# zenghjian/SceneSplat

Measured on AMD Instinct MI355X. Metric: Gaussians/s encoder fwd+bwd, 102k-pt chunks, higher is better.
Workload: dtype bf16

## Files before the change

### include/scenesplat_hip.h

```cpp
#ifndef SCENESPLAT_HIP_H
#define SCENESPLAT_HIP_H
#include <stddef.h>
#include <stdint.h>

#ifdef __cplusplus
extern "C" {
#endif

struct ihipStream_t;
typedef struct ihipStream_t* ss_stream_t;

#define SS_MAX_ORDERS 8
enum { SS_ORDER_Z = 0, SS_ORDER_Z_TRANS = 1, SS_ORDER_HILBERT = 2, SS_ORDER_HILBERT_TRANS = 3 };
enum { SS_DTYPE_F32 = 0, SS_DTYPE_BF16 = 1 };
enum { SS_ATTN_SIMT = 0, SS_ATTN_MFMA = 1 };

int ss_version(void);

int ss_serialize_encode(const int32_t* grid_coord, const int32_t* batch, int64_t n, int depth, const int* orders,
                        int num_orders, int64_t* codes, ss_stream_t stream);
int ss_offsets_to_batch(const int32_t* offsets, int num_batches, int64_t n, int32_t* batch, ss_stream_t stream);
int ss_count_duplicates(const int64_t* sorted_keys, int64_t n, int32_t* count, ss_stream_t stream);
int ss_grid_coord_max(const int32_t* grid_coord, int64_t n, int32_t* out_max, ss_stream_t stream);
size_t ss_argsort_workspace_bytes(int64_t n, int num_segments);
// ... 10 lines not shown
                        int32_t* grid_coord_out, int32_t* batch_out, int64_t* codes_out, ss_stream_t stream);
int ss_batch_offsets(const int32_t* batch, const int32_t* perm, int64_t n, int num_batches, int32_t* offsets,
                     ss_stream_t stream);

int ss_window_index(const int32_t* order, const int32_t* offsets, const int32_t* offsets_pad, int num_batches,
                    int patch_size, int64_t n_pad, int32_t* gidx, int32_t* sidx, ss_stream_t stream);
int ss_window_attn_fwd(const void* qkv, const int32_t* gidx, const int32_t* sidx, const int32_t* win_start,
                       int num_windows, int max_window, int64_t n, int64_t n_pad, int channels, int num_heads,
                       float scale, int dtype, int impl, void* out, float* lse, ss_stream_t stream);
size_t ss_window_attn_bwd_workspace_bytes(int64_t n, int64_t n_pad, int channels, int num_heads, int dtype);
int ss_window_attn_bwd(const void* qkv, const void* out, const void* dout, const float* lse, const int32_t* gidx,
                       const int32_t* sidx, const int32_t* win_start, int num_windows, int max_window, int64_t n,
                       int64_t n_pad, int channels, int num_heads, float scale, int dtype, int impl, void* dqkv,
                       void* workspace, size_t workspace_bytes, ss_stream_t stream);

int ss_cast_bf16_group(const int64_t* desc, const int32_t* wg_start, int nprob, int total_workgroups, ss_stream_t stream);
int ss_cast_bf16_group_elems_per_workgroup(void);

int ss_row_keep_scales(const int64_t* seed, const float* keep, float* out, int64_t n, ss_stream_t stream);

int ss_gelu(const void* x, const void* dy, void* out, int64_t numel, int dtype, ss_stream_t stream);

int ss_stream_capture_status(ss_stream_t stream);
unsigned long long ss_stream_capture_id(ss_stream_t stream);

int ss_linear_fwd_headmajor(const void* x, const int32_t* row_index, const void* weight, const float* bias, void* out_hm,
                            int64_t m, int k, int n_out, int channels, int head_dim, float sec0_scale, ss_stream_t stream);
int ss_headmajor_pack(const void* src, int in_dtype, const int32_t* gidx, void* hm, int64_t n_pad, int channels,
                      int num_heads, int sections, float sec0_scale, ss_stream_t stream);
int ss_window_attn_hm_fwd(const void* hm, const int32_t* sidx, const int32_t* win_start, int num_windows, int max_window,
                          int64_t n, int64_t n_pad, int channels, int num_heads, void* out, float* neg_lse2,
                          ss_stream_t stream);
size_t ss_window_attn_hm_bwd_workspace_bytes(int64_t n, int64_t n_pad, int channels, int num_heads);
int ss_window_attn_hm_bwd(const void* hm, const void* out, const void* dout, const float* neg_lse2, const int32_t* gidx,
                          const int32_t* sidx, const int32_t* win_start, int num_windows, int max_window, int64_t n,
                          int64_t n_pad, int channels, int num_heads, float scale, void* dqkv, void* workspace,
                          size_t workspace_bytes, ss_stream_t stream);

int ss_subm_rulebook(const int32_t* grid_coord, const int32_t* batch, int64_t n, int depth,
                     const int64_t* zkeys_sorted, const int32_t* zorder, int swap_xy, int kernel_size, int32_t* nbr,
                     ss_stream_t stream);
int ss_subm_tap_mask_keys(const int32_t* nbr, const int32_t* order, int64_t n, int taps, int coarse_bits, int64_t* keys,
                          ss_stream_t stream);
int64_t ss_subm_rulebook_table_size(int64_t n);
int ss_subm_rulebook_hashed(const int32_t* grid_coord, const int32_t* batch, int64_t n, int depth, int kernel_size, int32_t* nbr,
                            void* workspace, size_t workspace_bytes, ss_stream_t stream);

int ss_subm_conv_fwd(const void* in, const void* weight, const float* bias, const int32_t* nbr, const int32_t* rowperm,
                     void* out, int64_t n, int cin, int cout, int taps, int out_dtype, ss_stream_t stream);
int ss_subm_weight_mirror(const void* w, void* wt, int cout, int taps, int cin, ss_stream_t stream);
int ss_stream_create_cu_mask(int nwords, const uint32_t* mask, void** stream_out);
int ss_subm_im2col(const void* src, const int32_t* nbr, void* dst, int64_t n, int taps, int64_t row_bytes, ss_stream_t stream);
int ss_gemm8_ok(int64_t m, int k, int n, int taps);
int ss_subm_conv_fwd_pipe(const void* in, const void* weight, const float* bias, const int32_t* nbr, const int32_t* rowperm,
                          void* out, int64_t n, int cin, int cout, int taps, int out_dtype, ss_stream_t stream);
int ss_subm_conv_fwd_pipe_walk(const void* in, const void* weight, const float* bias, const int32_t* nbr_walk, const int32_t* rowperm,
                               void* out, int64_t n, int cin, int cout, int taps, int out_dtype, ss_stream_t stream);
int ss_subm_conv_fwd_uses_pipe(int64_t n, int cin, int cout, int taps);
int ss_subm_conv_fwd_walk(const void* in, const void* weight, const float* bias, const int32_t* nbr, const int32_t* nbr_walk,
                          const int32_t* rowperm, void* out, int64_t n, int cin, int cout, int taps, int out_dtype, ss_stream_t stream);
int ss_linear_fwd(const void* x, const void* weight, const float* bias, void* out, int64_t m, int k, int n, int out_dtype,
                  ss_stream_t stream);
int ss_wgrad_xcd_order(void);
int ss_wgrad_set_xcd_order(int on);
int ss_wgrad8_ok(int64_t n, int cin, int cout, int taps);
int ss_subm_conv_wgrad_pipe(const void* in, const void* dout, const int32_t* nbr, const int32_t* rowperm,
                            const int32_t* blk_count, const int32_t* blk_list, float* dweight, int64_t n, int cin, int cout,
                            int taps, ss_stream_t stream);
int ss_linear_wgrad(const void* x, const void* dy, float* dweight, float* dbias, int64_t m, int k_in, int n_out,
                    ss_stream_t stream);
int ss_linear_wgrad_group_plan(int64_t m, int k_in, int n_out, int64_t* desc_words);
int ss_linear_wgrad_tiles(int k_in, int n_out);
int ss_linear_wgrad_group_plan2(int64_t m, int k_in, int n_out, int launch_tiles, int64_t* desc_words);
int ss_linear_wgrad_group(const int64_t* desc, const int32_t* wg_start, int nprob, int total_workgroups, ss_stream_t stream);
int ss_subm_conv_splits(int64_t n, int cout, int taps);
int ss_subm_conv_fwd_splitk(const void* in, const void* weight, const float* bias, const int32_t* nbr, const int32_t* rowperm,
                            float* acc32, int64_t n, int cin, int cout, int taps, int splits, ss_stream_t stream);
int ss_subm_block_lists(const int32_t* nbr, const int32_t* rowperm, int64_t n, int taps, int32_t* blk_count,
                        int32_t* blk_list, ss_stream_t stream);
int ss_subm_conv_wgrad(const void* in, const void* dout, const int32_t* nbr, const int32_t* rowperm,
                       const int32_t* blk_count, const int32_t* blk_list, float* dweight, int64_t n, int cin, int cout,
                       int taps, ss_stream_t stream);

int ss_subm_f32_ok(int cin_padded, int cout);
int ss_subm_f32_fwd(const float* in, const float* wq, const float* bias, const int32_t* nbr_walk, const int32_t* rowperm,
                    float* out, int64_t n, int cin_padded, int cout, int taps, ss_stream_t stream);
int ss_subm_f32_dgrad_dup(const float* dout_folded, const float* wq, const int32_t* nbr_walk, const int32_t* rowperm, float* din,
                          int64_t n, int cin_padded, int cout, int taps, ss_stream_t stream);
int ss_subm_f32_wgrad(const float* in, const float* dout, const int32_t* nbr_walk, const int32_t* rowperm,
                      const int32_t* blk_count, const int32_t* blk_list, float* dweight, int64_t n, int cin_padded,
                      int cin, int cout, int taps, ss_stream_t stream);

int ss_subm_conv_wgrad_pipe_walk(const void* in, const void* dout, const int32_t* nbr_walk, const int32_t* rowperm,
                                 const int32_t* blk_count, const int32_t* blk_list, float* dweight, int64_t n, int cin, int cout,
                                 int taps, ss_stream_t stream);
int ss_subm_conv_wgrad_uses_pipe(int64_t n, int cin, int cout, int taps);
int ss_subm_conv_wgrad_walk(const void* in, const void* dout, const int32_t* nbr, const int32_t* nbr_walk, const int32_t* rowperm,
                            const int32_t* blk_count, const int32_t* blk_list, float* dweight, int64_t n, int cin, int cout,
                            int taps, ss_stream_t stream);

int ss_add_layernorm_fwd(const void* x, int x_dtype, const void* y, int y_dtype, const float* rowscale,
                         const float* gamma, const float* beta, float eps, void* xout, int xout_dtype, void* xcopy_bf16,
                         void* h, int h_dtype, float* mean, float* rstd, int64_t n, int channels, ss_stream_t stream);
int ss_ln_add_ln_fwd(const void* x, int x_dtype, const void* t, int t_dtype, const float* gamma0, const float* beta0, float eps0,
                     const float* gamma1, const float* beta1, float eps1, float* xout, void* h, int h_dtype, float* stats,
                     int64_t n, int channels, ss_stream_t stream);
// ... 117 lines not shown
```

### scenesplat_amd/_lib.py

```python
import ctypes
import os

import torch

_HERE = os.path.dirname(os.path.abspath(__file__))
LIB_PATH = os.path.join(_HERE, "lib", "libscenesplat_hip.so")

c_p = ctypes.c_void_p
c_i = ctypes.c_int
c_i64 = ctypes.c_int64
c_f = ctypes.c_float
c_sz = ctypes.c_size_t

PROTOTYPES = {
    "ss_version": (c_i, []),
    "ss_serialize_encode": (c_i, [c_p, c_p, c_i64, c_i, ctypes.POINTER(c_i), c_i, c_p, c_p]),
    "ss_offsets_to_batch": (c_i, [c_p, c_i, c_i64, c_p, c_p]),
    "ss_count_duplicates": (c_i, [c_p, c_i64, c_p, c_p]),
    "ss_grid_coord_max": (c_i, [c_p, c_i64, c_p, c_p]),
    "ss_argsort_workspace_bytes": (c_sz, [c_i64, c_i]),
    "ss_argsort_i64": (c_i, [c_p, c_i, c_i64, c_i, c_p, c_p, c_p, c_p, c_sz, c_p]),
    "ss_pool_partition_workspace_bytes": (c_sz, [c_i64]),
    "ss_pool_partition": (c_i, [c_p, c_p, c_i64, c_i, c_p, c_p, c_p, c_p, c_p, c_sz, c_p]),
    "ss_pool_level_attrs": (c_i, [c_p, c_i64, c_i64, c_p, c_p, c_p, c_i, c_i, c_p, c_p, c_p, c_p]),
    "ss_batch_offsets": (c_i, [c_p, c_p, c_i64, c_i, c_p, c_p]),
    "ss_window_index": (c_i, [c_p, c_p, c_p, c_i, c_i, c_i64, c_p, c_p, c_p]),
    "ss_window_attn_fwd": (c_i, [c_p, c_p, c_p, c_p, c_i, c_i, c_i64, c_i64, c_i, c_i, c_f, c_i, c_i, c_p, c_p, c_p]),
    "ss_window_attn_bwd_workspace_bytes": (c_sz, [c_i64, c_i64, c_i, c_i, c_i]),
    "ss_window_attn_bwd": (c_i, [c_p, c_p, c_p, c_p, c_p, c_p, c_p, c_i, c_i, c_i64, c_i64, c_i, c_i, c_f, c_i, c_i,
                                 c_p, c_p, c_sz, c_p]),
    "ss_gelu": (c_i, [c_p, c_p, c_p, c_i64, c_i, c_p]),
    "ss_row_keep_scales": (c_i, [c_p, c_p, c_p, c_i64, c_p]),
    "ss_stream_capture_status": (c_i, [c_p]),
    "ss_stream_capture_id": (ctypes.c_ulonglong, [c_p]),
    "ss_cast_bf16_group": (c_i, [c_p, c_p, c_i, c_i, c_p]),
    "ss_cast_bf16_group_elems_per_workgroup": (c_i, []),
    "ss_linear_fwd_headmajor": (c_i, [c_p, c_p, c_p, c_p, c_p, c_i64, c_i, c_i, c_i, c_i, c_f, c_p]),
    "ss_headmajor_pack": (c_i, [c_p, c_i, c_p, c_p, c_i64, c_i, c_i, c_i, c_f, c_p]),
    "ss_window_attn_hm_fwd": (c_i, [c_p, c_p, c_p, c_i, c_i, c_i64, c_i64, c_i, c_i, c_p, c_p, c_p]),
    "ss_window_attn_hm_bwd_workspace_bytes": (c_sz, [c_i64, c_i64, c_i, c_i]),
    "ss_window_attn_hm_bwd": (c_i, [c_p, c_p, c_p, c_p, c_p, c_p, c_p, c_i, c_i, c_i64, c_i64, c_i, c_i, c_f, c_p, c_p, c_sz, c_p]),
    "ss_subm_rulebook": (c_i, [c_p, c_p, c_i64, c_i, c_p, c_p, c_i, c_i, c_p, c_p]),
    "ss_subm_conv_fwd": (c_i, [c_p, c_p, c_p, c_p, c_p, c_p, c_i64, c_i, c_i, c_i, c_i, c_p]),
    "ss_stream_create_cu_mask": (c_i, [c_i, c_p, c_p]),
    "ss_ln_add_ln_fwd": (c_i, [c_p, c_i, c_p, c_i, c_p, c_p, c_f, c_p, c_p, c_f, c_p, c_p, c_i, c_p, c_i64, c_i, c_p]),
    "ss_ln_add_ln_bwd": (c_i, [c_p, c_p, c_i, c_p, c_p, c_i, c_p, c_p, c_p, c_p, c_i, c_p, c_i, c_p, c_i64, c_i, c_i, c_p]),
    "ss_segment_minmax": (c_i, [c_p, c_p, c_p, c_p, c_p, c_i64, c_i, c_i, c_i, c_p]),
    "ss_segment_minmax_bwd": (c_i, [c_p, c_p, c_p, c_i64, c_i, c_i, c_p]),
    "ss_subm_rulebook_table_size": (c_i64, [c_i64]),
    "ss_subm_rulebook_hashed": (c_i, [c_p, c_p, c_i64, c_i, c_i, c_p, c_p, ctypes.c_size_t, c_p]),
    "ss_subm_tap_mask_keys": (c_i, [c_p, c_p, c_i64, c_i, c_i, c_p, c_p]),
    "ss_subm_weight_mirror": (c_i, [c_p, c_p, c_i, c_i, c_i, c_p]),
    "ss_subm_im2col": (c_i, [c_p, c_p, c_p, c_i64, c_i, c_i64, c_p]),
    "ss_gemm8_ok": (c_i, [c_i64, c_i, c_i, c_i]),
    "ss_subm_conv_fwd_pipe": (c_i, [c_p, c_p, c_p, c_p, c_p, c_p, c_i64, c_i, c_i, c_i, c_i, c_p]),
    "ss_linear_fwd": (c_i, [c_p, c_p, c_p, c_p, c_i64, c_i, c_i, c_i, c_p]),
    "ss_wgrad_xcd_order": (c_i, []),
    "ss_wgrad_set_xcd_order": (c_i, [c_i]),
    "ss_wgrad8_ok": (c_i, [c_i64, c_i, c_i, c_i]),
    "ss_subm_conv_wgrad_pipe": (c_i, [c_p, c_p, c_p, c_p, c_p, c_p, c_p, c_i64, c_i, c_i, c_i, c_p]),
    "ss_linear_wgrad": (c_i, [c_p, c_p, c_p, c_p, c_i64, c_i, c_i, c_p]),
    "ss_linear_wgrad_group_plan": (c_i, [c_i64, c_i, c_i, c_p]),
    "ss_linear_wgrad_tiles": (c_i, [c_i, c_i]),
    "ss_linear_wgrad_group_plan2": (c_i, [c_i64, c_i, c_i, c_i, c_p]),
    "ss_linear_wgrad_group": (c_i, [c_p, c_p, c_i, c_i, c_p]),
    "ss_subm_conv_splits": (c_i, [c_i64, c_i, c_i]),
    "ss_subm_conv_fwd_splitk": (c_i, [c_p, c_p, c_p, c_p, c_p, c_p, c_i64, c_i, c_i, c_i, c_i, c_p]),
    "ss_subm_block_lists": (c_i, [c_p, c_p, c_i64, c_i, c_p, c_p, c_p]),
    "ss_subm_conv_wgrad": (c_i, [c_p, c_p, c_p, c_p, c_p, c_p, c_p, c_i64, c_i, c_i, c_i, c_p]),
    "ss_subm_conv_fwd_pipe_walk": (c_i, [c_p, c_p, c_p, c_p, c_p, c_p, c_i64, c_i, c_i, c_i, c_i, c_p]),
    "ss_subm_conv_fwd_uses_pipe": (c_i, [c_i64, c_i, c_i, c_i]),
    "ss_subm_conv_fwd_walk": (c_i, [c_p, c_p, c_p, c_p, c_p, c_p, c_p, c_i64, c_i, c_i, c_i, c_i, c_p]),
    "ss_subm_conv_wgrad_pipe_walk": (c_i, [c_p, c_p, c_p, c_p, c_p, c_p, c_p, c_i64, c_i, c_i, c_i, c_p]),
    "ss_subm_conv_wgrad_uses_pipe": (c_i, [c_i64, c_i, c_i, c_i]),
    "ss_subm_conv_wgrad_walk": (c_i, [c_p, c_p, c_p, c_p, c_p, c_p, c_p, c_p, c_i64, c_i, c_i, c_i, c_p]),
    "ss_subm_f32_ok": (c_i, [c_i, c_i]),
    "ss_subm_f32_fwd": (c_i, [c_p, c_p, c_p, c_p, c_p, c_p, c_i64, c_i, c_i, c_i, c_p]),
    "ss_subm_f32_dgrad_dup": (c_i, [c_p, c_p, c_p, c_p, c_p, c_i64, c_i, c_i, c_i, c_p]),
    "ss_dup_fold_rows": (c_i, [c_p, c_p, c_p, c_p, c_i64, c_i, c_i, c_p]),
    "ss_dup_zero_rows": (c_i, [c_p, c_p, c_p, c_i64, c_i64, c_p]),
    "ss_subm_f32_wgrad": (c_i, [c_p, c_p, c_p, c_p, c_p, c_p, c_p, c_i64, c_i, c_i, c_i, c_i, c_p]),
    "ss_add_layernorm_fwd": (c_i, [c_p, c_i, c_p, c_i, c_p, c_p, c_p, c_f, c_p, c_i, c_p, c_p, c_i, c_p, c_p, c_i64, c_i, c_p]),
    "ss_add_layernorm_bwd_blocks": (c_i, [c_i64]),
    "ss_group_partial_sums_outputs_per_workgroup": (c_i, []),
    "ss_group_partial_sums": (c_i, [c_p, c_p, c_i, c_i, c_p]),
    "ss_transpose16_group": (c_i, [c_p, c_p, c_i, c_i, c_p]),
    "ss_subm_weight_mirror_group_tile": (c_i, []),
    "ss_subm_weight_mirror_group": (c_i, [c_p, c_p, c_i, c_i, c_p]),
    "ss_add_layernorm_bwd": (c_i, [c_p, c_i, c_p, c_i, c_p, c_i, c_p, c_i, c_p, c_p, c_p, c_p, c_p, c_i, c_p, c_i, c_p, c_p,
                                   c_i64, c_i, c_i, c_p]),
    "ss_col_stats": (c_i, [c_p, c_i, c_p, c_p, c_p, c_i64, c_i, c_i, c_p]),
    "ss_bn_stats_finish": (c_i, [c_p, c_p, c_i, c_i, c_i64, c_f, c_f, c_p, c_p, c_p, c_p, c_p, c_p]),
    "ss_bn_bwd_finish": (c_i, [c_p, c_i, c_i, c_i64, c_p, c_p, c_p]),
    "ss_bn_act_fwd": (c_i, [c_p, c_i, c_p, c_p, c_p, c_p, c_i, c_p, c_i, c_i64, c_i, c_p]),
    "ss_bn_act_bwd_reduce": (c_i, [c_p, c_i, c_p, c_i, c_p, c_p, c_p, c_p, c_i, c_p, c_p, c_i64, c_i, c_i, c_p]),
    "ss_bn_act_bwd_apply": (c_i, [c_p, c_i, c_p, c_i, c_p, c_p, c_p, c_p, c_i, c_p, c_p, c_p, c_i, c_i64, c_i, c_p]),
    "ss_feat_text_scan": (c_i, [c_p, c_p, c_i64, c_i, c_i, c_p, c_p, c_p, c_p, c_p]),
    "ss_lang_head_blocks": (c_i, [c_i64]),
    "ss_lang_head_fwd": (c_i, [c_p, c_i, c_p, c_i, c_p, c_i, c_p, c_i, c_p, c_p, c_p, c_i64, c_i, c_p]),
    "ss_lang_head_bwd": (c_i, [c_p, c_i, c_p, c_i, c_p, c_i, c_p, c_p, c_p, c_i, c_p, c_i, c_i64, c_i, c_p]),
    "ss_seg_loss_workspace_bytes": (c_sz, [c_i64, c_i]),
    "ss_seg_loss_fwd": (c_i, [c_p, c_i, c_p, c_i64, c_i, c_i64, c_p, c_i, c_p, c_p, c_p, c_p, c_p, c_sz, c_p]),
    "ss_seg_loss_bwd": (c_i, [c_p, c_i, c_p, c_i64, c_i, c_i64, c_p, c_p, c_p, c_p, c_p, c_p]),
    "ss_seg_iou": (c_i, [c_p, c_i, c_p, c_p, c_i64, c_i, c_i64, c_p, c_p]),
    "ss_gather_rows": (c_i, [c_p, c_p, c_p, c_i64, c_i64, c_p]),
    "ss_scatter_rows": (c_i, [c_p, c_p, c_p, c_i64, c_i64, c_p]),
    "ss_gather_add_rows": (c_i, [c_p, c_p, c_p, c_p, c_i64, c_i, c_i, c_p]),
# ... 65 lines not shown
```

### scenesplat_amd/build.py

```python
import glob
import os
import subprocess
import sys

HERE = os.path.dirname(os.path.abspath(__file__))
CSRC = os.path.join(HERE, "csrc")
LIBDIR = os.path.join(HERE, "lib")
LIB = os.path.join(LIBDIR, "libscenesplat_hip.so")
HEADER = os.path.join(os.path.dirname(HERE), "include", "scenesplat_hip.h")


def sources():
    return sorted(glob.glob(os.path.join(CSRC, "*.hip")))


def _headers():
    return glob.glob(os.path.join(CSRC, "*.h")) + [HEADER]


def needs_build():
    if not os.path.exists(LIB):
        return True
    t = os.path.getmtime(LIB)
    return any(os.path.getmtime(d) > t for d in sources() + _headers())


def build(force=False, verbose=True):
    os.makedirs(LIBDIR, exist_ok=True)
    if os.environ.get("SS_EXTRA_HIPCC_FLAGS"):
        force = True
    if not force and not needs_build():
        return LIB
    hipcc = os.environ.get("HIPCC", "/opt/rocm/bin/hipcc")
    objdir = os.path.join(LIBDIR, "obj")
    os.makedirs(objdir, exist_ok=True)
    hdr_t = max(os.path.getmtime(h) for h in _headers())
    objs, procs = [], []
    for src in sources():
        obj = os.path.join(objdir, os.path.basename(src)[:-4] + ".o")
        objs.append(obj)
        if not force and os.path.exists(obj) and os.path.getmtime(obj) > max(os.path.getmtime(src), hdr_t):
            continue
        cmd = [hipcc, "--offload-arch=gfx950", "-O3", "-std=c++17", "-fPIC", "-c", src, "-o", obj,
               "-Wno-unused-value", "-Wno-unused-result",
               "-mllvm", "-amdgpu-mfma-vgpr-form"] + os.environ.get("SS_EXTRA_HIPCC_FLAGS", "").split()
        if verbose:
            print(" ".join(cmd), flush=True)
        procs.append((src, subprocess.Popen(cmd)))
    for src, p in procs:
        if p.wait() != 0:
            raise RuntimeError(f"hipcc failed on {src}")
    cmd = [hipcc, "--offload-arch=gfx950", "-shared", "-fPIC", "-o", LIB] + objs
    if verbose:
        print(" ".join(cmd), flush=True)
    subprocess.check_call(cmd)
    return LIB


if __name__ == "__main__":
    build(force="--force" in sys.argv)
```

### scenesplat_amd/csrc/gemm8.hip

```cpp
#include "common.h"
#include <stdlib.h>
#include "../../include/scenesplat_hip.h"

typedef __attribute__((ext_vector_type(8))) __bf16 g8_bf8_t;
#define G8_MFMA(a, b, c) __builtin_amdgcn_mfma_f32_16x16x32_bf16((a), (b), (c), 0, 0, 0)
#define G8_TAPS_MAX 27
#define G8_ZERO_ELEMS 4096

#ifndef G8_STAGGER
#define G8_STAGGER 1
#endif
#define G8_BUF 65536
#define G8_HALF 16384
#define G8_OFF_B 32768
#define G8_OFF_NBR 131072
#define G8_OFF_ROWID (G8_OFF_NBR + G8_TAPS_MAX * 256 * 4)
#define G8_OFF_MASK (G8_OFF_ROWID + 1024)
#define G8_LDS_BYTES (G8_OFF_MASK + 16)

__device__ uint4 g8_zero[G8_ZERO_ELEMS / 8];

__device__ __forceinline__ void g8_glds16(const void* gsrc, char* lds_wave_base) {
  __builtin_amdgcn_global_load_lds((const __attribute__((address_space(1))) void*)gsrc,
                                   (__attribute__((address_space(3))) void*)lds_wave_base, 16, 0, 0);
}
__device__ __forceinline__ g8_bf8_t g8_lds(const char* p) {
  return __builtin_bit_cast(g8_bf8_t, *reinterpret_cast<const uint4*>(p));
}

template <bool GATHER, typename OutT, bool HM = false>
__global__ void __launch_bounds__(512)
k_gemm8(const unsigned short* __restrict__ A, const unsigned short* __restrict__ W, const float* __restrict__ bias,
        const int32_t* __restrict__ nbr, const int32_t* __restrict__ rowperm, OutT* __restrict__ out, int M, int K,
        int N, int taps, int ntn, int hm_c = 0, int hm_d = 0, float hm_scale = 1.f, int walk = 0) {
  __shared__ __attribute__((aligned(16))) char smem[G8_LDS_BYTES];
  int32_t* nbr_s = reinterpret_cast<int32_t*>(smem + G8_OFF_NBR);
  int32_t* rowid_s = reinterpret_cast<int32_t*>(smem + G8_OFF_ROWID);
  unsigned* mask_s = reinterpret_cast<unsigned*>(smem + G8_OFF_MASK);
  const int tid = threadIdx.x, wave = tid >> 6, lane = tid & 63, lq = lane & 15, g = lane >> 4;
  const int wr = wave >> 2, wc = wave & 3;
  int L;
  {
    const int nwg = gridDim.x, orig = blockIdx.x, xcd = orig & 7, q = nwg >> 3, r = nwg & 7;
    L = (xcd < r ? xcd * (q + 1) : r * (q + 1) + (xcd - r) * q) + (orig >> 3);
  }
  const int m0 = (L / ntn) * 256, n0 = (L % ntn) * 256;

  unsigned rem = 0u;
  int tap = 0;
  if (GATHER) {
    if (tid < 256) {
      int k = m0 + tid;
      rowid_s[tid] = k < M ? (rowperm ? rowperm[k] : k) : -1;
    }
    if (tid == 0) *mask_s = 0u;
// ... 174 lines not shown
    asm volatile("s_waitcnt vmcnt(0)" ::: "memory");
  }

  int64_t hm_base[2][2];
  float hm_mul[2][2];
  if (HM) {
#pragma unroll
    for (int hb = 0; hb < 2; ++hb)
#pragma unroll
      for (int ni = 0; ni < 2; ++ni) {
        const int col = min(n0 + 64 * wc + 32 * hb + 16 * ni + 4 * g, N - 4);
        const int sec = col / hm_c, cc = col - sec * hm_c, hd = cc / hm_d, dd = cc - hd * hm_d;
        hm_base[hb][ni] = ((int64_t)sec * (hm_c / hm_d) + hd) * M * hm_d + dd;
        hm_mul[hb][ni] = sec == 0 ? hm_scale : 1.f;
      }
  }
#pragma unroll
  for (int ha = 0; ha < 2; ++ha)
#pragma unroll
    for (int mi = 0; mi < 4; ++mi) {
      const int R = 128 * wr + 64 * ha + 16 * mi + lq;
      int64_t row;
      if (GATHER) { row = rowid_s[R]; } else { row = m0 + R < M ? m0 + R : -1; }
      if (row < 0) continue;
#pragma unroll
      for (int hb = 0; hb < 2; ++hb)
#pragma unroll
        for (int ni = 0; ni < 2; ++ni) {
          const int col = n0 + 64 * wc + 32 * hb + 16 * ni + 4 * g;
          if (col >= N) continue;
          f32x4_t v = acc[ha][mi][hb][ni];
          if (bias) { float4 bv = *reinterpret_cast<const float4*>(bias + col); v[0] += bv.x; v[1] += bv.y; v[2] += bv.z; v[3] += bv.w; }
          OutT* op = out + row * N + col;
          if (HM) {
            const float m_ = hm_mul[hb][ni];
            v[0] *= m_; v[1] *= m_; v[2] *= m_; v[3] *= m_;
            op = out + hm_base[hb][ni] + row * hm_d;
          }
          if (sizeof(OutT) == 2) {
            uint2 u; u.x = pack_bf16x2(v[0], v[1]); u.y = pack_bf16x2(v[2], v[3]);
            *reinterpret_cast<uint2*>(op) = u;
          } else {
            *reinterpret_cast<float4*>(op) = make_float4(v[0], v[1], v[2], v[3]);
          }
        }
    }
}

extern "C" int ss_gemm8_ok(int64_t m, int k, int n, int taps) {
  return m > 0 && m < (1LL << 31) && k >= 64 && (k & 63) == 0 && k <= G8_ZERO_ELEMS && n >= 4 && (n & 3) == 0 &&
         taps >= 1 && taps <= G8_TAPS_MAX;
}

template <bool GATHER>
static int g8_launch(const void* a, const void* w, const float* bias, const int32_t* nbr, const int32_t* rowperm, void* out,
                     int64_t m, int k, int n, int taps, int out_dtype, hipStream_t stream, int walk = 0) {
  if (!ss_gemm8_ok(m, k, n, taps)) return SS_ERR_ARG;
  const int ntm = ss_div_up(m, 256), ntn = ss_div_up(n, 256);
  dim3 grid(ntm * ntn), block(512);
  const unsigned short* A = (const unsigned short*)a; const unsigned short* Wp = (const unsigned short*)w;
  if (out_dtype == SS_BF16)
    SS_LAUNCH((k_gemm8<GATHER, unsigned short>), grid, block, 0, stream, A, Wp, bias, nbr, rowperm, (unsigned short*)out, (int)m, k, n, taps, ntn, 0, 0, 1.f, walk);
  else if (out_dtype == SS_F32)
    SS_LAUNCH((k_gemm8<GATHER, float>), grid, block, 0, stream, A, Wp, bias, nbr, rowperm, (float*)out, (int)m, k, n, taps, ntn, 0, 0, 1.f, walk);
  else
    return SS_ERR_ARG;
  return SS_OK;
}

extern "C" int ss_subm_conv_fwd_pipe(const void* in, const void* weight, const float* bias, const int32_t* nbr,
                                     const int32_t* rowperm, void* out, int64_t n, int cin, int cout, int taps,
                                     int out_dtype, hipStream_t stream) {
  if (n == 0) return SS_OK;
  return g8_launch<true>(in, weight, bias, nbr, rowperm, out, n, cin, cout, taps, out_dtype, stream);
}

extern "C" int ss_subm_conv_fwd_pipe_walk(const void* in, const void* weight, const float* bias, const int32_t* nbr_walk,
                                          const int32_t* rowperm, void* out, int64_t n, int cin, int cout, int taps,
                                          int out_dtype, hipStream_t stream) {
  if (n == 0) return SS_OK;
  return g8_launch<true>(in, weight, bias, nbr_walk, rowperm, out, n, cin, cout, taps, out_dtype, stream, 1);
}

extern "C" int ss_linear_fwd(const void* x, const void* weight, const float* bias, void* out, int64_t m, int k, int n,
                             int out_dtype, hipStream_t stream) {
  if (m == 0) return SS_OK;
  return g8_launch<false>(x, weight, bias, nullptr, nullptr, out, m, k, n, 1, out_dtype, stream);
}

extern "C" int ss_linear_fwd_headmajor(const void* x, const int32_t* row_index, const void* weight, const float* bias,
                                       void* out_hm, int64_t m, int k, int n_out, int channels, int head_dim,
                                       float sec0_scale, hipStream_t stream) {
  if (m == 0) return SS_OK;
  if (!ss_gemm8_ok(m, k, n_out, 1) || channels <= 0 || head_dim <= 0 || (head_dim & 3) || channels % head_dim || n_out % channels ||
      !row_index)
    return SS_ERR_ARG;
  const int ntm = ss_div_up(m, 256), ntn = ss_div_up(n_out, 256);
  dim3 grid(ntm * ntn), block(512);
  SS_LAUNCH((k_gemm8<false, unsigned short, true>), grid, block, 0, stream, (const unsigned short*)x, (const unsigned short*)weight,
            bias, (const int32_t*)nullptr, row_index, (unsigned short*)out_hm, (int)m, k, n_out, 1, ntn, channels, head_dim,
            sec0_scale);
  return SS_OK;
}
```

### scenesplat_amd/native.py

```python
import ctypes
import os

import torch

from . import _lib
from ._lib import check

F32, BF16 = 0, 1
ATTN_SIMT, ATTN_MFMA = 0, 1
HAVE_MFMA_ATTN = True
ORDER_IDS = {"z": 0, "z-trans": 1, "hilbert": 2, "hilbert-trans": 3}


_GROUP_WIDE_SHARES = os.environ.get("SS_WGRAD_GROUP_WIDE", "1") != "0"
_GROUP_KEEP = []
_GROUP_LOCK = __import__("threading").Lock()


class DescriptorPool:

    def __init__(self, nbytes=1 << 20):
        self.buf = torch.empty(int(nbytes), dtype=torch.uint8).pin_memory()
        self.off = 0
        self.device_side = []
# ... 195 lines not shown
    return keys


def subm_conv_fwd_uses_pipe(n, cin, cout, taps):
    return bool(lib().ss_subm_conv_fwd_uses_pipe(n, cin, cout, taps)) and lib().ss_subm_conv_splits(n, cout, taps) <= 1


def subm_conv_fwd(x, w, bias, nbr, rowperm, out_dtype=torch.bfloat16, nbr_walk=None):
    n, cin = x.shape
    cout, taps, cin2 = w.shape
    _req(x, torch.bfloat16, "x"); _req(w, torch.bfloat16, "w"); _req(nbr, torch.int32, "nbr", (taps, n))
    if cin2 != cin or cin % 8:
        raise RuntimeError(f"subm_conv_fwd: cin mismatch / not a multiple of 8 ({cin}, {cin2})")
    if bias is not None:
        _req(bias, torch.float32, "bias", (cout,))
    if rowperm is not None:
        _req(rowperm, torch.int32, "rowperm", (n,))
    splits = lib().ss_subm_conv_splits(n, cout, taps)
    if splits > 1:
        acc = torch.zeros((n, cout), dtype=torch.float32, device=x.device)
        check(lib().ss_subm_conv_fwd_splitk(_p(x), _p(w), _p(bias), _p(nbr), _p(rowperm), _p(acc), n, cin, cout, taps, splits,
                                            _stream()), "ss_subm_conv_fwd_splitk")
        return acc if out_dtype == torch.float32 else acc.to(out_dtype)
    out = torch.empty((n, cout), dtype=out_dtype, device=x.device)
    if nbr_walk is not None:
        _req(nbr_walk, torch.int32, "nbr_walk", (taps, n))
        check(lib().ss_subm_conv_fwd_walk(_p(x), _p(w), _p(bias), _p(nbr), _p(nbr_walk), _p(rowperm), _p(out), n, cin, cout, taps,
                                          dtype_code(out), _stream()), "ss_subm_conv_fwd_walk")
        return out
    check(lib().ss_subm_conv_fwd(_p(x), _p(w), _p(bias), _p(nbr), _p(rowperm), _p(out), n, cin, cout, taps,
                                 dtype_code(out), _stream()), "ss_subm_conv_fwd")
    return out


def subm_weight_mirror(w):
    cout, taps, cin = w.shape
    _req(w, torch.bfloat16, "w")
    wt = torch.empty((cin, taps, cout), dtype=torch.bfloat16, device=w.device)
    check(lib().ss_subm_weight_mirror(_p(w), _p(wt), cout, taps, cin, _stream()), "ss_subm_weight_mirror")
    return wt


def subm_im2col(x, nbr):
    n, c = x.shape
    taps = nbr.shape[0]
    _req(x, torch.bfloat16, "x"); _req(nbr, torch.int32, "nbr", (taps, n))
    if c % 8:
        raise RuntimeError("subm_im2col: channels must be a multiple of 8")
    out = torch.empty((n, taps * c), dtype=torch.bfloat16, device=x.device)
    check(lib().ss_subm_im2col(_p(x), _p(nbr), _p(out), n, taps, c * 2, _stream()), "ss_subm_im2col")
    return out


def subm_conv_fwd_pipe(x, w, bias, nbr, rowperm, out_dtype=torch.bfloat16):
    n, cin = x.shape
    cout, taps = w.shape[0], w.shape[1]
    out = torch.empty((n, cout), dtype=out_dtype, device=x.device)
    check(lib().ss_subm_conv_fwd_pipe(_p(x), _p(w), _p(bias), _p(nbr), _p(rowperm), _p(out), n, cin, cout, taps,
                                      dtype_code(out), _stream()), "ss_subm_conv_fwd_pipe")
    return out


def linear_fwd(x, w, bias=None, out_dtype=torch.bfloat16):
    m, k = x.shape
    n = w.shape[0]
    out = torch.empty((m, n), dtype=out_dtype, device=x.device)
    check(lib().ss_linear_fwd(_p(x), _p(w), _p(bias), _p(out), m, k, n, dtype_code(out), _stream()), "ss_linear_fwd")
    return out


def subm_block_lists(nbr, rowperm):
    taps, n = nbr.shape
    _req(nbr, torch.int32, "nbr")
    if rowperm is not None:
        _req(rowperm, torch.int32, "rowperm", (n,))
    nb = (n + 63) // 64
    cnt = torch.empty(taps, dtype=torch.int32, device=nbr.device)
    lst = torch.empty((taps, nb), dtype=torch.int32, device=nbr.device)
    check(lib().ss_subm_block_lists(_p(nbr), _p(rowperm), n, taps, _p(cnt), _p(lst), _stream()), "ss_subm_block_lists")
    return cnt, lst


_ARENA = {"buf": None, "off": 0}


def zero_arena_begin(numel, device):
    _ARENA["buf"] = torch.zeros(int(numel), dtype=torch.float32, device=device) if numel > 0 else None
    _ARENA["off"] = 0


def zeros_f32(numel, device):
    buf, off = _ARENA["buf"], _ARENA["off"]
    if buf is not None and buf.device == device and off + numel <= buf.numel():
        _ARENA["off"] = off + ((numel + 3) & ~3)
        return buf[off:off + numel]
    return torch.zeros(int(numel), dtype=torch.float32, device=device)


def subm_conv_wgrad(x, dout, nbr, rowperm, blocks, out=None, nbr_walk=None):
    n, cin = x.shape
    cout = dout.shape[1]
    taps = nbr.shape[0]
    _req(x, torch.bfloat16, "x"); _req(dout, torch.bfloat16, "dout", (n, cout)); _req(nbr, torch.int32, "nbr", (taps, n))
    if cin % 8 or cout % 8:
        raise RuntimeError("subm_conv_wgrad: channels must be multiples of 8")
    if rowperm is not None:
        _req(rowperm, torch.int32, "rowperm", (n,))
    dw = zeros_f32(cout * taps * cin, x.device).view(cout, taps, cin) if out is None else _req(out, torch.float32, "out", (cout, taps, cin))
    cnt, lst = blocks
    _req(cnt, torch.int32, "blk_count", (taps,)); _req(lst, torch.int32, "blk_list", (taps, (n + 63) // 64))
    if nbr_walk is not None:
        _req(nbr_walk, torch.int32, "nbr_walk", (taps, n))
    check(lib().ss_subm_conv_wgrad_walk(_p(x), _p(dout), _p(nbr), _p(nbr_walk), _p(rowperm), _p(cnt), _p(lst), _p(dw), n, cin, cout, taps,
# ... 655 lines not shown
```

Before: 2.827 million.

## Add 4-wave 256x256 gemm8 variant with AGPR accumulators for large convs

Adds a new 256-thread (4-wave) GEMM kernel in which each wave holds a 128x128 accumulator tile in AGPRs. It uses a hand-scheduled double-buffered LDS pipeline with global_load_lds DMA interleaved between MFMAs, and the file is compiled without the VGPR-form MFMA flag. By default, gathered sparse-conv forward calls with m>=25600 and k>=512 go to the new kernel; other calls can be forced to 4 or 8 waves through an env var or setter. The aim is to cut LDS and synchronisation overhead per MFMA and to improve latency hiding in the big conv GEMMs. The cost is heavy register pressure and a fragile, hand-tuned schedule.

```diff
diff --git a/include/scenesplat_hip.h b/include/scenesplat_hip.h
--- a/include/scenesplat_hip.h
+++ b/include/scenesplat_hip.h
@@ -86,6 +86,8 @@
 int ss_stream_create_cu_mask(int nwords, const uint32_t* mask, void** stream_out);
 int ss_subm_im2col(const void* src, const int32_t* nbr, void* dst, int64_t n, int taps, int64_t row_bytes, ss_stream_t stream);
 int ss_gemm8_ok(int64_t m, int k, int n, int taps);
+int ss_gemm8_waves(void);
+int ss_gemm8_set_waves(int waves);
 int ss_subm_conv_fwd_pipe(const void* in, const void* weight, const float* bias, const int32_t* nbr, const int32_t* rowperm,
                           void* out, int64_t n, int cin, int cout, int taps, int out_dtype, ss_stream_t stream);
 int ss_subm_conv_fwd_pipe_walk(const void* in, const void* weight, const float* bias, const int32_t* nbr_walk, const int32_t* rowperm,
diff --git a/scenesplat_amd/_lib.py b/scenesplat_amd/_lib.py
--- a/scenesplat_amd/_lib.py
+++ b/scenesplat_amd/_lib.py
@@ -53,6 +53,8 @@
     "ss_subm_weight_mirror": (c_i, [c_p, c_p, c_i, c_i, c_i, c_p]),
     "ss_subm_im2col": (c_i, [c_p, c_p, c_p, c_i64, c_i, c_i64, c_p]),
     "ss_gemm8_ok": (c_i, [c_i64, c_i, c_i, c_i]),
+    "ss_gemm8_waves": (c_i, []),
+    "ss_gemm8_set_waves": (c_i, [c_i]),
     "ss_subm_conv_fwd_pipe": (c_i, [c_p, c_p, c_p, c_p, c_p, c_p, c_i64, c_i, c_i, c_i, c_i, c_p]),
     "ss_linear_fwd": (c_i, [c_p, c_p, c_p, c_p, c_i64, c_i, c_i, c_i, c_p]),
     "ss_wgrad_xcd_order": (c_i, []),
diff --git a/scenesplat_amd/build.py b/scenesplat_amd/build.py
--- a/scenesplat_amd/build.py
+++ b/scenesplat_amd/build.py
@@ -8,6 +8,9 @@
 LIBDIR = os.path.join(HERE, "lib")
 LIB = os.path.join(LIBDIR, "libscenesplat_hip.so")
 HEADER = os.path.join(os.path.dirname(HERE), "include", "scenesplat_hip.h")
+
+
+AGPR_FORM = {"gemm8w4.hip"}
 
 
 def sources():
@@ -42,8 +45,10 @@
         if not force and os.path.exists(obj) and os.path.getmtime(obj) > max(os.path.getmtime(src), hdr_t):
             continue
         cmd = [hipcc, "--offload-arch=gfx950", "-O3", "-std=c++17", "-fPIC", "-c", src, "-o", obj,
-               "-Wno-unused-value", "-Wno-unused-result",
-               "-mllvm", "-amdgpu-mfma-vgpr-form"] + os.environ.get("SS_EXTRA_HIPCC_FLAGS", "").split()
+               "-Wno-unused-value", "-Wno-unused-result"]
+        if os.path.basename(src) not in AGPR_FORM:
+            cmd += ["-mllvm", "-amdgpu-mfma-vgpr-form"]
+        cmd += os.environ.get("SS_EXTRA_HIPCC_FLAGS", "").split()
         if verbose:
             print(" ".join(cmd), flush=True)
         procs.append((src, subprocess.Popen(cmd)))
diff --git a/scenesplat_amd/csrc/gemm8.hip b/scenesplat_amd/csrc/gemm8.hip
--- a/scenesplat_amd/csrc/gemm8.hip
+++ b/scenesplat_amd/csrc/gemm8.hip
@@ -1,6 +1,7 @@
 #include "common.h"
 #include <stdlib.h>
 #include "../../include/scenesplat_hip.h"
+#include "gemm8w4.h"
 
 typedef __attribute__((ext_vector_type(8))) __bf16 g8_bf8_t;
 #define G8_MFMA(a, b, c) __builtin_amdgcn_mfma_f32_16x16x32_bf16((a), (b), (c), 0, 0, 0)
@@ -281,10 +282,30 @@
          taps >= 1 && taps <= G8_TAPS_MAX;
 }
 
+enum { G8_CLS_CONV = 0, G8_CLS_PLAIN = 1, G8_CLS_HM = 2 };
+static int g8_waves_mode = -1;
+extern "C" int ss_gemm8_waves(void) {
+  if (g8_waves_mode < 0) { const char* e = getenv("SS_GEMM8_WAVES"); const int v = e ? atoi(e) : 0; g8_waves_mode = (v == 4 || v == 8) ? v : 0; }
+  return g8_waves_mode;
+}
+extern "C" int ss_gemm8_set_waves(int waves) {
+  if (waves != 0 && waves != 4 && waves != 8) return SS_ERR_ARG;
+  g8_waves_mode = waves;
+  return SS_OK;
+}
+static bool g8_use_w4(int cls, int64_t m, int k, int n) {
+  const int mode = ss_gemm8_waves();
+  if (mode) return mode == 4;
+  (void)n;
+  return cls == G8_CLS_CONV && m >= 25600 && k >= 512;
+}
+
 template <bool GATHER>
 static int g8_launch(const void* a, const void* w, const float* bias, const int32_t* nbr, const int32_t* rowperm, void* out,
                      int64_t m, int k, int n, int taps, int out_dtype, hipStream_t stream, int walk = 0) {
   if (!ss_gemm8_ok(m, k, n, taps)) return SS_ERR_ARG;
+  if (g8_use_w4(GATHER ? G8_CLS_CONV : G8_CLS_PLAIN, m, k, n))
+    return g8w4_launch(GATHER, a, w, bias, nbr, rowperm, out, m, k, n, taps, out_dtype, stream, walk);
   const int ntm = ss_div_up(m, 256), ntn = ss_div_up(n, 256);
   dim3 grid(ntm * ntn), block(512);
   const unsigned short* A = (const unsigned short*)a; const unsigned short* Wp = (const unsigned short*)w;
@@ -324,6 +345,8 @@
   if (!ss_gemm8_ok(m, k, n_out, 1) || channels <= 0 || head_dim <= 0 || (head_dim & 3) || channels % head_dim || n_out % channels ||
       !row_index)
     return SS_ERR_ARG;
+  if (g8_use_w4(G8_CLS_HM, m, k, n_out))
+    return g8w4_launch_headmajor(x, row_index, weight, bias, out_hm, m, k, n_out, channels, head_dim, sec0_scale, stream);
   const int ntm = ss_div_up(m, 256), ntn = ss_div_up(n_out, 256);
   dim3 grid(ntm * ntn), block(512);
   SS_LAUNCH((k_gemm8<false, unsigned short, true>), grid, block, 0, stream, (const unsigned short*)x, (const unsigned short*)weight,
diff --git a/scenesplat_amd/csrc/gemm8w4.h b/scenesplat_amd/csrc/gemm8w4.h
--- /dev/null
+++ b/scenesplat_amd/csrc/gemm8w4.h
@@ -0,0 +1,7 @@
+#pragma once
+#include "common.h"
+
+int g8w4_launch(int gather, const void* a, const void* w, const float* bias, const int32_t* nbr, const int32_t* rowperm,
+                void* out, int64_t m, int k, int n, int taps, int out_dtype, hipStream_t stream, int walk);
+int g8w4_launch_headmajor(const void* x, const int32_t* row_index, const void* weight, const float* bias, void* out_hm,
+                          int64_t m, int k, int n_out, int channels, int head_dim, float sec0_scale, hipStream_t stream);
diff --git a/scenesplat_amd/csrc/gemm8w4.hip b/scenesplat_amd/csrc/gemm8w4.hip
--- /dev/null
+++ b/scenesplat_amd/csrc/gemm8w4.hip
@@ -0,0 +1,292 @@
+#include "common.h"
+#include "gemm8w4.h"
+
+typedef __attribute__((ext_vector_type(8))) __bf16 g4_bf8_t;
+#define G4_MFMA(a, b, c) __builtin_amdgcn_mfma_f32_16x16x32_bf16((a), (b), (c), 0, 0, 0)
+#define G4_TAPS_MAX 27
+#define G4_ZERO_ELEMS 4096
+#define G4_BUF 65536
+#define G4_HALF 16384
+#define G4_OFF_B 32768
+#define G4_OFF_NBR 131072
+#define G4_OFF_ROWID (G4_OFF_NBR + G4_TAPS_MAX * 256 * 4)
+#define G4_OFF_MASK (G4_OFF_ROWID + 1024)
+#define G4_LDS_BYTES (G4_OFF_MASK + 16)
+
+__device__ uint4 g4_zero[G4_ZERO_ELEMS / 8];
+
+__device__ __forceinline__ void g4_glds16(const void* gsrc, char* lds_wave_base) {
+  __builtin_amdgcn_global_load_lds((const __attribute__((address_space(1))) void*)gsrc,
+                                   (__attribute__((address_space(3))) void*)lds_wave_base, 16, 0, 0);
+}
+__device__ __forceinline__ g4_bf8_t g4_lds(const char* p) {
+  return __builtin_bit_cast(g4_bf8_t, *reinterpret_cast<const uint4*>(p));
+}
+#ifndef G4_DMA_EVERY
+#define G4_DMA_EVERY 4
+#endif
+#ifndef G4_X_AT
+#define G4_X_AT 16
+#endif
+#ifndef G4_RD_EVERY
+#define G4_RD_EVERY 2
+#endif
+#define G4_X_ISSUED ((G4_X_AT + G4_DMA_EVERY - 1) / G4_DMA_EVERY)
+#define G4_X_INFLIGHT (G4_X_ISSUED < 16 ? G4_X_ISSUED : 16)
+#define G4_PIN() __builtin_amdgcn_sched_barrier(0)
+#ifdef G4_DIAG_NOBAR
+#define G4_BAR_X() G4_PIN()
+#else
+#define G4_BAR_X() G4_BAR()
+#endif
+#define G4_BAR() do { G4_PIN(); __builtin_amdgcn_s_barrier(); G4_PIN(); } while (0)
+
+template <bool GATHER, typename OutT, bool HM = false>
+__global__ void __launch_bounds__(256)
+k_gemm8w4(const unsigned short* __restrict__ A, const unsigned short* __restrict__ W, const float* __restrict__ bias,
+          const int32_t* __restrict__ nbr, const int32_t* __restrict__ rowperm, OutT* __restrict__ out, int M, int K,
+          int N, int taps, int ntn, int hm_c = 0, int hm_d = 0, float hm_scale = 1.f, int walk = 0) {
+  __shared__ __attribute__((aligned(16))) char smem[G4_LDS_BYTES];
+  int32_t* nbr_s = reinterpret_cast<int32_t*>(smem + G4_OFF_NBR);
+  int32_t* rowid_s = reinterpret_cast<int32_t*>(smem + G4_OFF_ROWID);
+  unsigned* mask_s = reinterpret_cast<unsigned*>(smem + G4_OFF_MASK);
+  const int tid = threadIdx.x, wave = tid >> 6, lane = tid & 63, lq = lane & 15, g = lane >> 4;
+  const int wr = wave >> 1, wc = wave & 1;
+  int L;
+  {
+    const int nwg = gridDim.x, orig = blockIdx.x, xcd = orig & 7, q = nwg >> 3, r = nwg & 7;
+    L = (xcd < r ? xcd * (q + 1) : r * (q + 1) + (xcd - r) * q) + (orig >> 3);
+  }
+  const int m0 = (L / ntn) * 256, n0 = (L % ntn) * 256;
+
+  unsigned rem = 0u;
+  int tap = 0;
+  if (GATHER) {
+    {
+      int k = m0 + tid;
+      rowid_s[tid] = k < M ? (rowperm ? rowperm[k] : k) : -1;
+    }
+    if (tid == 0) *mask_s = 0u;
+    __syncthreads();
+    int vals[G4_TAPS_MAX];
+    const int myrow = rowid_s[tid];
+    const int32_t* const src = nbr + (walk ? min(m0 + tid, M - 1) : max(myrow, 0));
+#pragma unroll
+    for (int it = 0; it < G4_TAPS_MAX; ++it) vals[it] = src[(int64_t)min(it, taps - 1) * M];
+#pragma unroll
+    for (int it = 0; it < G4_TAPS_MAX; ++it) vals[it] = myrow >= 0 ? vals[it] : -1;
+#pragma unroll
+    for (int it = 0; it < G4_TAPS_MAX; ++it) {
+      if (it < taps) {
+        nbr_s[it * 256 + tid] = vals[it];
+        if (__ballot(vals[it] >= 0) != 0ULL && lane == 0) atomicOr(mask_s, 1u << it);
+      }
+    }
+    __syncthreads();
+    rem = __builtin_amdgcn_readfirstlane(*mask_s);
+  }
+  const int ksteps = K >> 6;
+  int T;
+  if (GATHER) {
+    T = __builtin_popcount(rem) * ksteps;
+    if (rem) { tap = __builtin_ctz(rem); rem &= rem - 1u; }
+    else T = 1;
+  } else {
+    T = ksteps;
+  }
+
+  f32x4_t acc[8][8];
+
+  const int lc8 = (((tid & 7) ^ ((tid >> 4) & 7)) << 3);
+  const int srow = tid >> 3;
+  const unsigned short* pA[2][4];
+  const unsigned short* pB[2][4];
+  auto load_rows = [&](int tp) {
+#pragma unroll
+    for (int h = 0; h < 2; ++h)
+#pragma unroll
+      for (int jj = 0; jj < 4; ++jj) {
+        int R = 128 * (jj >> 1) + 64 * h + 32 * (jj & 1) + srow;
+        if (GATHER) {
+          const int src = nbr_s[tp * 256 + R];
+          const unsigned short* const row = A + (int64_t)max(src, 0) * K;
+          pA[h][jj] = (src >= 0 ? row : reinterpret_cast<const unsigned short*>(g4_zero)) + lc8;
+        } else {
+          int row = min(m0 + R, M - 1);
+          if (HM) row = rowperm[row];
+          pA[h][jj] = A + (int64_t)row * K + lc8;
+        }
+      }
+  };
+#pragma unroll
+  for (int h = 0; h < 2; ++h)
+#pragma unroll
+    for (int jj = 0; jj < 4; ++jj) {
+      int col = min(n0 + 64 * jj + 32 * h + srow, N - 1);
+      pB[h][jj] = W + (int64_t)col * taps * K + lc8;
+    }
+  int kc = 0;
+  int64_t boff = (int64_t)tap * K;
+  load_rows(tap);
+  int staged = 0;
+  auto advance = [&]() {
+    if (staged + 1 >= T) return;
+    ++staged;
+    kc += 64;
+    if (GATHER) {
+      if (kc == K) {
+        kc = 0;
+        tap = __builtin_ctz(rem); rem &= rem - 1u;
+        boff = (int64_t)tap * K;
+        load_rows(tap);
+      }
+    } else if (kc == K) {
+      kc = 0;
+    }
+  };
+  char* const dst0 = smem + __builtin_amdgcn_readfirstlane(wave) * 1024;
+  auto stage1 = [&](char* bufbase, int i) {
+    const int h = (i >> 2) & 1, jj = i & 3;
+    if (i < 8) g4_glds16(pA[h][jj] + kc, bufbase + h * G4_HALF + jj * 4096);
+    else g4_glds16(pB[h][jj] + boff + kc, bufbase + G4_OFF_B + h * G4_HALF + jj * 4096);
+  };
+
+  const int sw = (lq >> 1) & 7;
+  const int oA = (wr * 64 + lq) * 128 + ((g ^ sw) << 4);
+  const int oB = G4_OFF_B + (wc * 64 + lq) * 128 + ((g ^ sw) << 4);
+  g4_bf8_t fa[2][8], fb[2][8];
+#define G4_READ(BASE, KS, I)                                                                                        \
+  do {                                                                                                              \
+    if ((I) < 8) fb[KS][(I)&7] = g4_lds((BASE) + (((I) >> 1) & 1) * G4_HALF + (oB ^ ((KS) * 64)) +                  \
+                                        ((((I)&7) >> 2) * 32 + ((I)&1) * 16) * 128);                                \
+    else fa[KS][(I)&7] = g4_lds((BASE) + (((I)&7) >> 2) * G4_HALF + (oA ^ ((KS) * 64)) + ((I)&3) * 2048);           \
+  } while (0)
+#define G4_MM(KS, MI) acc[(MI) >> 3][(MI)&7] = G4_MFMA(fb[KS][(MI)&7], fa[KS][(MI) >> 3], acc[(MI) >> 3][(MI)&7])
+
+  {
+#pragma unroll
+    for (int i = 0; i < 16; ++i) stage1(dst0, i);
+    advance();
+#pragma unroll
+    for (int i = 0; i < 16; ++i) stage1(dst0 + G4_BUF, i);
+    asm volatile("s_waitcnt vmcnt(16)" ::: "memory");
+    G4_BAR();
+#pragma unroll
+    for (int i = 0; i < 16; ++i) G4_READ(smem, 0, i);
+    G4_PIN();
+#pragma unroll
+    for (int i = 0; i < 8; ++i)
+#pragma unroll
+      for (int j = 0; j < 8; ++j) {
+        acc[i][j] = f32x4_t{0.f, 0.f, 0.f, 0.f};
+        asm volatile("" : "+a"(acc[i][j]));
+      }
+    G4_PIN();
+    for (int t = 0; t < T; ++t) {
+      const int bo = (t & 1) * G4_BUF;
+      const char* const cur = smem + bo;
+      const char* const nxt = smem + (bo ^ G4_BUF);
+#pragma unroll
+      for (int m = 0; m < 64; ++m) {
+        if (m % 3 == 0 && m / 3 < 16) G4_READ(cur, 1, m / 3);
+        G4_MM(0, m);
+        G4_PIN();
+      }
+      asm volatile("s_waitcnt lgkmcnt(0)" ::: "memory");
+      if (G4_X_AT == 0) asm volatile("s_waitcnt vmcnt(0)" ::: "memory");
+      G4_BAR_X();
+      advance();
+      G4_PIN();
+#pragma unroll
+      for (int m = 0; m < 64; ++m) {
+        if (G4_X_AT > 0 && m == G4_X_AT) {
+          G4_PIN();
+          asm volatile("s_waitcnt vmcnt(%0)" ::"n"(G4_X_INFLIGHT) : "memory");
+          G4_BAR_X();
+        }
+#ifndef G4_DIAG_NODMA
+        if (m % G4_DMA_EVERY == 0 && m / G4_DMA_EVERY < 16) stage1(dst0 + bo, m / G4_DMA_EVERY);
+#endif
+        if (m >= G4_X_AT && (m - G4_X_AT) % G4_RD_EVERY == 0 && (m - G4_X_AT) / G4_RD_EVERY < 16) G4_READ(nxt, 0, (m - G4_X_AT) / G4_RD_EVERY);
+        G4_MM(1, m);
+        G4_PIN();
+      }
+    }
+    asm volatile("s_waitcnt vmcnt(0)" ::: "memory");
+  }
+
+  int64_t hm_base[8];
+  float hm_mul[8];
+  if (HM) {
+#pragma unroll
+    for (int j = 0; j < 8; ++j) {
+      const int col = min(n0 + 128 * wc + 16 * j + 4 * g, N - 4);
+      const int sec = col / hm_c, cc = col - sec * hm_c, hd = cc / hm_d, dd = cc - hd * hm_d;
+      hm_base[j] = ((int64_t)sec * (hm_c / hm_d) + hd) * M * hm_d + dd;
+      hm_mul[j] = sec == 0 ? hm_scale : 1.f;
+    }
+  }
+  float4 bv[8];
+#pragma unroll
+  for (int j = 0; j < 8; ++j)
+    bv[j] = bias ? *reinterpret_cast<const float4*>(bias + min(n0 + 128 * wc + 16 * j + 4 * g, N - 4)) : make_float4(0.f, 0.f, 0.f, 0.f);
+#pragma unroll
+  for (int i = 0; i < 8; ++i) {
+    const int R = 128 * wr + 16 * i + lq;
+    int64_t row;
+    if (GATHER) { row = rowid_s[R]; } else { row = m0 + R < M ? m0 + R : -1; }
+#pragma unroll
+    for (int j = 0; j < 8; ++j) asm volatile("" : "+a"(acc[i][j])::"memory");
+    G4_PIN();
+    if (row < 0) continue;
+#pragma unroll
+    for (int j = 0; j < 8; ++j) {
+      const int col = n0 + 128 * wc + 16 * j + 4 * g;
+      if (col >= N) continue;
+      f32x4_t v = acc[i][j];
+      if (bias) { v[0] += bv[j].x; v[1] += bv[j].y; v[2] += bv[j].z; v[3] += bv[j].w; }
+      OutT* op = out + row * N + col;
+      if (HM) {
+        const float m_ = hm_mul[j];
+        v[0] *= m_; v[1] *= m_; v[2] *= m_; v[3] *= m_;
+        op = out + hm_base[j] + row * hm_d;
+      }
+      if (sizeof(OutT) == 2) {
+        uint2 u; u.x = pack_bf16x2(v[0], v[1]); u.y = pack_bf16x2(v[2], v[3]);
+        *reinterpret_cast<uint2*>(op) = u;
+      } else {
+        *reinterpret_cast<float4*>(op) = make_float4(v[0], v[1], v[2], v[3]);
+      }
+    }
+  }
+}
+
+int g8w4_launch(int gather, const void* a, const void* w, const float* bias, const int32_t* nbr, const int32_t* rowperm,
+                void* out, int64_t m, int k, int n, int taps, int out_dtype, hipStream_t stream, int walk) {
+  const int ntm = ss_div_up(m, 256), ntn = ss_div_up(n, 256);
+  dim3 grid(ntm * ntn), block(256);
+  const unsigned short* A = (const unsigned short*)a; const unsigned short* Wp = (const unsigned short*)w;
+  if (out_dtype != SS_BF16 && out_dtype != SS_F32) return SS_ERR_ARG;
+  if (gather) {
+    if (out_dtype == SS_BF16)
+      SS_LAUNCH((k_gemm8w4<true, unsigned short>), grid, block, 0, stream, A, Wp, bias, nbr, rowperm, (unsigned short*)out, (int)m, k, n, taps, ntn, 0, 0, 1.f, walk);
+    else
+      SS_LAUNCH((k_gemm8w4<true, float>), grid, block, 0, stream, A, Wp, bias, nbr, rowperm, (float*)out, (int)m, k, n, taps, ntn, 0, 0, 1.f, walk);
+  } else {
+    if (out_dtype == SS_BF16)
+      SS_LAUNCH((k_gemm8w4<false, unsigned short>), grid, block, 0, stream, A, Wp, bias, nbr, rowperm, (unsigned short*)out, (int)m, k, n, taps, ntn, 0, 0, 1.f, walk);
+    else
+      SS_LAUNCH((k_gemm8w4<false, float>), grid, block, 0, stream, A, Wp, bias, nbr, rowperm, (float*)out, (int)m, k, n, taps, ntn, 0, 0, 1.f, walk);
+  }
+  return SS_OK;
+}
+
+int g8w4_launch_headmajor(const void* x, const int32_t* row_index, const void* weight, const float* bias, void* out_hm,
+                          int64_t m, int k, int n_out, int channels, int head_dim, float sec0_scale, hipStream_t stream) {
+  const int ntm = ss_div_up(m, 256), ntn = ss_div_up(n_out, 256);
+  dim3 grid(ntm * ntn), block(256);
+  SS_LAUNCH((k_gemm8w4<false, unsigned short, true>), grid, block, 0, stream, (const unsigned short*)x, (const unsigned short*)weight,
+            bias, (const int32_t*)nullptr, row_index, (unsigned short*)out_hm, (int)m, k, n_out, 1, ntn, channels, head_dim,
+            sec0_scale, 0);
+  return SS_OK;
+}
diff --git a/scenesplat_amd/native.py b/scenesplat_amd/native.py
--- a/scenesplat_amd/native.py
+++ b/scenesplat_amd/native.py
@@ -271,13 +271,21 @@
     return out
 
 
-def subm_conv_fwd_pipe(x, w, bias, nbr, rowperm, out_dtype=torch.bfloat16):
+def subm_conv_fwd_pipe(x, w, bias, nbr, rowperm, out_dtype=torch.bfloat16, walk=False):
     n, cin = x.shape
     cout, taps = w.shape[0], w.shape[1]
     out = torch.empty((n, cout), dtype=out_dtype, device=x.device)
-    check(lib().ss_subm_conv_fwd_pipe(_p(x), _p(w), _p(bias), _p(nbr), _p(rowperm), _p(out), n, cin, cout, taps,
-                                      dtype_code(out), _stream()), "ss_subm_conv_fwd_pipe")
-    return out
+    fn, name = (lib().ss_subm_conv_fwd_pipe_walk, "ss_subm_conv_fwd_pipe_walk") if walk else (lib().ss_subm_conv_fwd_pipe, "ss_subm_conv_fwd_pipe")
+    check(fn(_p(x), _p(w), _p(bias), _p(nbr), _p(rowperm), _p(out), n, cin, cout, taps, dtype_code(out), _stream()), name)
+    return out
+
+
+def gemm8_set_waves(waves):
+    check(lib().ss_gemm8_set_waves(int(waves)), "ss_gemm8_set_waves")
+
+
+def gemm8_waves():
+    return lib().ss_gemm8_waves()
 
 
 def linear_fwd(x, w, bias=None, out_dtype=torch.bfloat16):
```

Measured after the change: 2.841 million (median of 6 runs). No clear change (+0.5%).
